# aapdo/M3ViT

Measured on AMD Instinct MI355X. Metric: images/sec fwd+bwd ViT-S/16 MoE(E=16,k=4) 224^2 bs=128, higher is better.
Workload: dtype f16; 1 GPU; configs[1]: ViT-Small/16 + MoE E=16 top-k=4 multi_gate, synthetic 224x224; batch_per_gpu=128, global_batch=128, task_passes=2, launch=hipGraph replay (one linear graph per task pass and stream), routing=deterministic (std=0), task_streams=2, wgrad_streams=0, activation_checkpointing=False, parallelism=single, full=False

## Files before the change

### m3vit_amd/csrc/attention_b16.hip

```cpp
#include "attention_dev.h"
#include <type_traits>

namespace m3 {

constexpr int AR_THREADS = 256;
constexpr float AR_LOG2E = 1.4426950408889634f;

typedef __fp16 ar_fp16x4 __attribute__((__vector_size__(4 * sizeof(__fp16))));

template <int W> __device__ __forceinline__ int swo(int row, int byte) {
  if (W == 32) return row * 64 + ((((byte >> 4) ^ (row >> 1)) & 3) << 4) + (byte & 15);
  return row * 128 + ((((byte >> 4) ^ row) & 7) << 4) + (byte & 15);
}

template <typename T, int W> __device__ __forceinline__ typename Mma<T>::frag row_frag(const char *img, int r0, int ch, int li, int lg) {
  return *(const typename Mma<T>::frag *)(img + swo<W>(r0 + li, ch * 64 + lg * 16));
}

template <typename T, int W> __device__ __forceinline__ typename Mma<T>::frag tr_frag(const char *img, int rb, int col, int li, int lg) {
  const int r = rb + 4 * lg + (li >> 2), byte = (col + 4 * (li & 3)) * 2;
  const ar_fp16x4 lo = __builtin_amdgcn_ds_read_tr16_b64_v4f16((__attribute__((address_space(3))) ar_fp16x4 *)(img + swo<W>(r, byte)));
  const ar_fp16x4 hi = __builtin_amdgcn_ds_read_tr16_b64_v4f16((__attribute__((address_space(3))) ar_fp16x4 *)(img + swo<W>(r + 16, byte)));
  f16x8 f;
  f[0] = (half_t)lo[0]; f[1] = (half_t)lo[1]; f[2] = (half_t)lo[2]; f[3] = (half_t)lo[3];
  f[4] = (half_t)hi[0]; f[5] = (half_t)hi[1]; f[6] = (half_t)hi[2]; f[7] = (half_t)hi[3];
  return __builtin_bit_cast(typename Mma<T>::frag, f);
}


template <typename T, int DH, int NKT>
__global__ __launch_bounds__(AR_THREADS, DH == 32 ? 4 : 2) void attention_fwd_res_kernel(const T *__restrict__ qkv, int N, int heads,
                                                                           T *__restrict__ o,
                                                                           float *__restrict__ lse, float scale) {
  constexpr int RBY = DH * 2, CPR = RBY / 16, NCH = DH / 32, NDT = DH / 16;
  constexpr int NKEY = NKT * 16, NQW = NKT / 4;
  extern __shared__ __attribute__((aligned(16))) char smem[];
  char *sK = smem, *sV = smem + NKEY * RBY;

  const int tid = threadIdx.x, lane = tid & 63, wave = tid >> 6;
  const int li = lane & 15, lg = lane >> 4;
  const int bh = xcd_remap(blockIdx.x, gridDim.x), b = bh / heads, h = bh - b * heads;
  const int C = heads * DH;
  const int64_t ld = 3 * (int64_t)C;
  const T *qbase = qkv + (int64_t)b * N * ld + h * DH;
  const T *kbase = qbase + C, *vbase = qbase + 2 * C;

  const int nkt = (N + 15) >> 4;
  typename Mma<T>::frag qfs[NQW][NCH];
#pragma unroll
  for (int i = 0; i < NQW; ++i) {
    const int qrow = (i * 4 + wave) * 16 + li;
#pragma unroll
    for (int ch = 0; ch < NCH; ++ch) {
      qfs[i][ch] = Mma<T>::zero();
      if (qrow < N) qfs[i][ch] = *(const typename Mma<T>::frag *)(qbase + (int64_t)qrow * ld + ch * 32 + 8 * lg);
    }
  }
  {
    constexpr int SIT = NKEY * CPR / AR_THREADS;
    constexpr int SB = SIT % 4 == 0 ? 4 : (SIT % 3 == 0 ? 3 : (SIT % 2 == 0 ? 2 : 1));
#pragma unroll
    for (int it0 = 0; it0 < SIT; it0 += SB) {
      u32x4 kv[SB], vv[SB];
#pragma unroll
      for (int it = 0; it < SB; ++it) {
        const int q = (it0 + it) * AR_THREADS + tid, row = q / CPR, c = q % CPR;
        kv[it] = u32x4{0u, 0u, 0u, 0u}; vv[it] = kv[it];
        if (row < N) {
          kv[it] = *(const u32x4 *)((const char *)(kbase + (int64_t)row * ld) + c * 16);
          vv[it] = *(const u32x4 *)((const char *)(vbase + (int64_t)row * ld) + c * 16);
        }
      }
#pragma unroll
      for (int it = 0; it < SB; ++it) {
        const int q = (it0 + it) * AR_THREADS + tid, row = q / CPR, c = q % CPR;
        *(u32x4 *)(sK + swo<DH>(row, c * 16)) = kv[it];
        *(u32x4 *)(sV + swo<DH>(row, c * 16)) = vv[it];
      }
    }
  }
  __syncthreads();

  const float c1 = scale * AR_LOG2E;
  const f32x4 zero4 = f32x4{0.f, 0.f, 0.f, 0.f};
#pragma unroll
  for (int i = 0; i < NQW; ++i) {
    const int qt = i * 4 + wave;
    if (qt >= nkt) break;
    const int qrow = qt * 16 + li;
    f32x4 st[NKT];
    float mx = -INFINITY;
#pragma unroll
    for (int kt = 0; kt < NKT; ++kt) {
      f32x4 sv = zero4;
#pragma unroll
      for (int ch = 0; ch < NCH; ++ch) sv = Mma<T>::mma(row_frag<T, DH>(sK, kt * 16, ch, li, lg), qfs[i][ch], sv);
      if (kt >= NKT - 4) {
#pragma unroll
        for (int r = 0; r < 4; ++r) sv[r] = (kt * 16 + 4 * lg + r < N) ? sv[r] : -INFINITY;
      }
      mx = fmaxf(fmaxf(mx, fmaxf(sv[0], sv[1])), fmaxf(sv[2], sv[3]));
      st[kt] = sv;
    }
    mx = fmaxf(mx, __shfl_xor(mx, 16, 64));
    mx = fmaxf(mx, __shfl_xor(mx, 32, 64));
    const float mc = mx * c1;
    float psum = 0.f;
#pragma unroll
    for (int kt = 0; kt < NKT; ++kt) {
#pragma unroll
      for (int r = 0; r < 4; ++r) {
        const float p = __builtin_amdgcn_exp2f(st[kt][r] * c1 - mc);
        st[kt][r] = p;
        psum += p;
      }
    }
    psum += __shfl_xor(psum, 16, 64);
    psum += __shfl_xor(psum, 32, 64);
    f32x4 oacc[NDT];
#pragma unroll
    for (int dt = 0; dt < NDT; ++dt) oacc[dt] = zero4;
#pragma unroll
    for (int cc = 0; cc < NKT / 2; ++cc) {
      const typename Mma<T>::frag pf = Mma<T>::from_tiles(&st[cc * 2]);
#pragma unroll
      for (int dt = 0; dt < NDT; ++dt) oacc[dt] = Mma<T>::mma(tr_frag<T, DH>(sV, cc * 32, dt * 16, li, lg), pf, oacc[dt]);
    }
    if (qrow < N) {
      const float inv = 1.0f / psum;
      T *orow = o + ((int64_t)b * N + qrow) * C + h * DH;
#pragma unroll
      for (int dt = 0; dt < NDT; ++dt) Vec4<T>::store(orow + dt * 16 + 4 * lg, oacc[dt] * inv);
      if (lg == 0) lse[((int64_t)b * heads + h) * N + qrow] = mx * scale + __logf(psum);
    }
  }
}

#ifdef M3_ATTN_STAMPS
constexpr int ASTAMP_WGS = 2048, ASTAMP_N = 40;
__device__ unsigned long long g_attn_stamps[ASTAMP_WGS][ASTAMP_N];
#define ATTN_STAMP(i)                                                                              \
  do {                                                                                             \
    if (threadIdx.x == 0 && blockIdx.x < ASTAMP_WGS && (i) < ASTAMP_N) g_attn_stamps[blockIdx.x][(i)] = __builtin_amdgcn_s_memtime(); \
  } while (0)
#else
#define ATTN_STAMP(i) do { } while (0)
#endif

template <typename T, int DH, int KTE>
__global__ __launch_bounds__(DH == 32 ? 256 : 512, DH == 32 ? 2 : 1) void attention_bwd_res_kernel(
    const T *__restrict__ qkv, const T *__restrict__ o, const T *__restrict__ d_o,
    const float *__restrict__ lse, int N, int heads, T *__restrict__ dqkv, float scale) {
  constexpr int RBY = DH * 2, CPR = RBY / 16, NCH = DH / 32, NDT = DH / 16;
  constexpr int NW = DH == 32 ? 4 : 8, NT = NW * 64;
  constexpr int NKEY = KTE * NW * 16, NKC = NKEY / 32;
  static_assert(2 * NDT == NW, "one dQ piece per wave");
  static_assert(NKEY <= ATTN_KEYS, "at most 256 keys");
  extern __shared__ __attribute__((aligned(16))) char smem[];
  const int NP = (N + 31) & ~31;
  char *sQ = smem, *sdO = sQ + NP * RBY, *sK = sdO + NP * RBY;
  char *sdS = sK + NKEY * RBY;
  float *sLse = (float *)(sdS + 2 * NKEY * 64);
  float *sDelta = sLse + NP;

  const int tid = threadIdx.x, lane = tid & 63, wave = __builtin_amdgcn_readfirstlane(tid >> 6);
  const int li = lane & 15, lg = lane >> 4;
  const int bh = xcd_remap(blockIdx.x, gridDim.x), b = bh / heads, h = bh - b * heads;
  const int C = heads * DH;
  const int64_t ld = 3 * (int64_t)C;
  const T *qbase = qkv + (int64_t)b * N * ld + h * DH;
  const T *kbase = qbase + C, *vbase = qbase + 2 * C;
  const T *obase = o + (int64_t)b * N * C + h * DH;
  const T *dobase = d_o + (int64_t)b * N * C + h * DH;
  T *dqbase = dqkv + (int64_t)b * N * ld + h * DH;
  const float *lbase = lse + ((int64_t)b * heads + h) * N;
  ATTN_STAMP(0);

  {
    constexpr int SIT = NKEY * CPR / NT;
    u32x4 qv[SIT], dv[SIT], kv[SIT], ov[SIT];
    float lv[SIT];
#pragma unroll
    for (int it = 0; it < SIT; ++it) {
      const int q = it * NT + tid, row = q / CPR, c = q % CPR;
      qv[it] = u32x4{0u, 0u, 0u, 0u}; dv[it] = qv[it]; kv[it] = qv[it]; ov[it] = qv[it];
      lv[it] = 1e30f;
      if (row < N) {
        qv[it] = *(const u32x4 *)((const char *)(qbase + (int64_t)row * ld) + c * 16);
        kv[it] = *(const u32x4 *)((const char *)(kbase + (int64_t)row * ld) + c * 16);
        dv[it] = *(const u32x4 *)((const char *)(dobase + (int64_t)row * C) + c * 16);
        ov[it] = *(const u32x4 *)((const char *)(obase + (int64_t)row * C) + c * 16);
        if (c == 0) lv[it] = lbase[row] * AR_LOG2E;
      }
    }
#pragma unroll
    for (int it = 0; it < SIT; ++it) {
      const int q = it * NT + tid, row = q / CPR, c = q % CPR;
      const typename Mma<T>::frag dh8 = __builtin_bit_cast(typename Mma<T>::frag, dv[it]), oh8 = __builtin_bit_cast(typename Mma<T>::frag, ov[it]);
      float sd = 0.f;
#pragma unroll
      for (int j = 0; j < 8; ++j) sd += (float)dh8[j] * (float)oh8[j];
#pragma unroll
      for (int m = 1; m < CPR; m <<= 1) sd += __shfl_xor(sd, m, 64);
      *(u32x4 *)(sK + swo<DH>(row, c * 16)) = kv[it];
      if (row < NP) {
        *(u32x4 *)(sQ + swo<DH>(row, c * 16)) = qv[it];
        *(u32x4 *)(sdO + swo<DH>(row, c * 16)) = dv[it];
        if (c == 0) {
          sDelta[row] = sd;
          sLse[row] = lv[it];
        }
      }
    }
  }
  typename Mma<T>::frag kf[KTE][NCH], vf[KTE][NCH];
#pragma unroll
  for (int kt = 0; kt < KTE; ++kt) {
    const int key = (kt * NW + wave) * 16 + li;
#pragma unroll
    for (int ch = 0; ch < NCH; ++ch) {
      kf[kt][ch] = Mma<T>::zero();
      vf[kt][ch] = Mma<T>::zero();
      if (key < N) {
        kf[kt][ch] = *(const typename Mma<T>::frag *)(kbase + (int64_t)key * ld + ch * 32 + 8 * lg);
        vf[kt][ch] = *(const typename Mma<T>::frag *)(vbase + (int64_t)key * ld + ch * 32 + 8 * lg);
      }
    }
  }
  const f32x4 zero4 = f32x4{0.f, 0.f, 0.f, 0.f};
  f32x4 dkt[NDT][KTE], dvt[NDT][KTE];
#pragma unroll
  for (int a = 0; a < NDT; ++a)
#pragma unroll
    for (int c = 0; c < KTE; ++c) { dkt[a][c] = zero4; dvt[a][c] = zero4; }
  ATTN_STAMP(1);
  __syncthreads();
  ATTN_STAMP(2);

  const float c1 = scale * AR_LOG2E, inv_c1 = 1.0f / c1;
  const int nsteps = NP >> 5;
  const bool last_key_ok = ((KTE - 1) * NW + wave) * 16 + li < N;
  const int dq_qt = wave / NDT, dq_dt = wave - dq_qt * NDT;
  typename Mma<T>::frag ka[NKC];
#pragma unroll
  for (int c = 0; c < NKC; ++c) ka[c] = tr_frag<T, DH>(sK, c * 32, dq_dt * 16, li, lg);
  for (int st = 0; st < nsteps; ++st) {
    const int qs = st * 32;
    char *dsb = sdS + (st & 1) * NKEY * 64;
    f32x4 pt[2][KTE], dst[2][KTE];
#pragma unroll
    for (int qt = 0; qt < 2; ++qt) {
      typename Mma<T>::frag qfr[NCH], dof[NCH];
#pragma unroll
      for (int ch = 0; ch < NCH; ++ch) {
        qfr[ch] = row_frag<T, DH>(sQ, qs + qt * 16, ch, li, lg);
        dof[ch] = row_frag<T, DH>(sdO, qs + qt * 16, ch, li, lg);
      }
      const f32x4 l4 = *(const f32x4 *)(sLse + qs + qt * 16 + 4 * lg), d4 = *(const f32x4 *)(sDelta + qs + qt * 16 + 4 * lg);
      const f32x4 s0 = l4 * (-inv_c1), dp0 = -d4;
#pragma unroll
      for (int kt = 0; kt < KTE; ++kt) {
        f32x4 s = s0, dp = dp0;
#pragma unroll
        for (int ch = 0; ch < NCH; ++ch) {
          s = Mma<T>::mma(qfr[ch], kf[kt][ch], s);
          dp = Mma<T>::mma(dof[ch], vf[kt][ch], dp);
        }
        f32x4 pv;
#pragma unroll
        for (int r = 0; r < 4; ++r) pv[r] = __builtin_amdgcn_exp2f(s[r] * c1);
        if (kt == KTE - 1) {
#pragma unroll
          for (int r = 0; r < 4; ++r) pv[r] = last_key_ok ? pv[r] : 0.f;
        }
        pt[qt][kt] = pv;
        dst[qt][kt] = pv * dp;
      }
    }
    ATTN_STAMP(3 + 4 * st);
    {
      typename Mma<T>::frag aq[NDT], ado[NDT];
#pragma unroll
      for (int dt = 0; dt < NDT; ++dt) {
        aq[dt] = tr_frag<T, DH>(sQ, qs, dt * 16, li, lg);
        ado[dt] = tr_frag<T, DH>(sdO, qs, dt * 16, li, lg);
      }
#pragma unroll
      for (int kt = 0; kt < KTE; ++kt) {
        f32x4 tp[2] = {pt[0][kt], pt[1][kt]}, td[2] = {dst[0][kt], dst[1][kt]};
        const typename Mma<T>::frag pf = Mma<T>::from_tiles(tp), dsf = Mma<T>::from_tiles(td);
#pragma unroll
        for (int dt = 0; dt < NDT; ++dt) {
          dvt[dt][kt] = Mma<T>::mma(ado[dt], pf, dvt[dt][kt]);
          dkt[dt][kt] = Mma<T>::mma(aq[dt], dsf, dkt[dt][kt]);
        }
        const int krow = (kt * NW + wave) * 16 + li;
#pragma unroll
        for (int qt = 0; qt < 2; ++qt) {
          typename Vec4<T>::type v = typename Vec4<T>::type{(T)dst[qt][kt][0], (T)dst[qt][kt][1], (T)dst[qt][kt][2], (T)dst[qt][kt][3]};
          *(typename Vec4<T>::type *)(dsb + swo<32>(krow, (qt * 16 + 4 * lg) * 2)) = v;
        }
      }
    }
    ATTN_STAMP(4 + 4 * st);
    __syncthreads();
    ATTN_STAMP(5 + 4 * st);
    {
      typename Mma<T>::frag da[NKC];
#pragma unroll
      for (int c = 0; c < NKC; ++c) da[c] = tr_frag<T, 32>(dsb, c * 32, dq_qt * 16, li, lg);
      f32x4 acc = zero4, acc2 = zero4;
#pragma unroll
      for (int c = 0; c < NKC; c += 2) {
        acc = Mma<T>::mma(ka[c], da[c], acc);
        if (c + 1 < NKC) acc2 = Mma<T>::mma(ka[c + 1], da[c + 1], acc2);
      }
      acc += acc2;
      const int qr = qs + dq_qt * 16 + li;
      if (qr < N) Vec4<T>::store(dqbase + (int64_t)qr * ld + dq_dt * 16 + 4 * lg, acc * scale);
    }
    ATTN_STAMP(6 + 4 * st);
  }

#pragma unroll
  for (int kt = 0; kt < KTE; ++kt) {
    const int key = (kt * NW + wave) * 16 + li;
    if (key < N) {
#pragma unroll
      for (int dt = 0; dt < NDT; ++dt) {
        Vec4<T>::store(dqbase + C + (int64_t)key * ld + dt * 16 + 4 * lg, dkt[dt][kt] * scale);
        Vec4<T>::store(dqbase + 2 * C + (int64_t)key * ld + dt * 16 + 4 * lg, dvt[dt][kt]);
      }
    }
  }
  ATTN_STAMP(36);
#ifdef M3_ATTN_STAMPS
  asm volatile("s_waitcnt vmcnt(0)" ::: "memory");
  ATTN_STAMP(37);
#endif
}

template <typename T, int DH>
__global__ __launch_bounds__(AR_THREADS, 2) void attention_fwd_stream_kernel(const T *__restrict__ qkv, int N, int heads,
                                                                              T *__restrict__ o,
                                                                              float *__restrict__ lse, float scale) {
  constexpr int RBY = DH * 2, CPR = RBY / 16, NCH = DH / 32, NDT = DH / 16;
  constexpr int KT = 64;
  constexpr int NLD = KT * CPR / AR_THREADS;
  extern __shared__ __attribute__((aligned(16))) char smem[];
  char *sK = smem, *sV = smem + 2 * KT * RBY;

  const int tid = threadIdx.x, lane = tid & 63, wave = tid >> 6;
  const int li = lane & 15, lg = lane >> 4;
  const int nqb = gridDim.x;
  const int log_id = xcd_remap(blockIdx.x + nqb * blockIdx.y, nqb * gridDim.y);
  const int qb = log_id % nqb;
  const int bh = log_id / nqb, b = bh / heads, h = bh - b * heads;
  const int C = heads * DH;
  const int64_t ld = 3 * (int64_t)C;
  const T *qbase = qkv + (int64_t)b * N * ld + h * DH;
  const T *kbase = qbase + C, *vbase = qbase + 2 * C;

  const int qrow = qb * 64 + wave * 16 + li;
  typename Mma<T>::frag qf[NCH];
#pragma unroll
  for (int ch = 0; ch < NCH; ++ch) {
    qf[ch] = Mma<T>::zero();
    if (qrow < N) qf[ch] = *(const typename Mma<T>::frag *)(qbase + (int64_t)qrow * ld + ch * 32 + 8 * lg);
  }
  u32x4 rk[NLD], rv[NLD];
  auto fetch = [&](int key0) {
#pragma unroll
    for (int i = 0; i < NLD; ++i) {
      const int q = tid + AR_THREADS * i, row = q / CPR, c = q % CPR;
      rk[i] = u32x4{0u, 0u, 0u, 0u};
      rv[i] = u32x4{0u, 0u, 0u, 0u};
      if (key0 + row < N) {
        rk[i] = *(const u32x4 *)((const char *)(kbase + (int64_t)(key0 + row) * ld) + c * 16);
        rv[i] = *(const u32x4 *)((const char *)(vbase + (int64_t)(key0 + row) * ld) + c * 16);
      }
    }
  };
  auto stash = [&](int buf) {
#pragma unroll
    for (int i = 0; i < NLD; ++i) {
      const int q = tid + AR_THREADS * i, row = q / CPR, c = q % CPR;
      *(u32x4 *)(sK + buf * KT * RBY + swo<DH>(row, c * 16)) = rk[i];
      *(u32x4 *)(sV + buf * KT * RBY + swo<DH>(row, c * 16)) = rv[i];
    }
  };
  fetch(0);
  stash(0);
  __syncthreads();

  const f32x4 zero4 = f32x4{0.f, 0.f, 0.f, 0.f};
  f32x4 oacc[NDT];
#pragma unroll
  for (int dt = 0; dt < NDT; ++dt) oacc[dt] = zero4;
  const float c1 = scale * AR_LOG2E;
  float m_run = -INFINITY, l_run = 0.f;
  const int ntiles = (N + KT - 1) / KT;
  for (int t = 0; t < ntiles; ++t) {
    const int key0 = t * KT, buf = t & 1;
    const bool more = t + 1 < ntiles;
    if (more) fetch(key0 + KT);
    const char *cK = sK + buf * KT * RBY, *cV = sV + buf * KT * RBY;
    f32x4 st[4];
    float mt = -INFINITY;
#pragma unroll
    for (int kt = 0; kt < 4; ++kt) {
      f32x4 sv = zero4;
#pragma unroll
      for (int ch = 0; ch < NCH; ++ch) sv = Mma<T>::mma(row_frag<T, DH>(cK, kt * 16, ch, li, lg), qf[ch], sv);
      if (!more) {
#pragma unroll
        for (int r = 0; r < 4; ++r) sv[r] = (key0 + kt * 16 + 4 * lg + r < N) ? sv[r] : -INFINITY;
      }
      mt = fmaxf(fmaxf(mt, fmaxf(sv[0], sv[1])), fmaxf(sv[2], sv[3]));
      st[kt] = sv;
    }
    mt = fmaxf(mt, __shfl_xor(mt, 16, 64));
    mt = fmaxf(mt, __shfl_xor(mt, 32, 64));
    const float m_new = fmaxf(m_run, mt);
    const float alpha = __builtin_amdgcn_exp2f((m_run - m_new) * c1);
    const float mc = m_new * c1;
    float psum = 0.f;
#pragma unroll
    for (int kt = 0; kt < 4; ++kt)
#pragma unroll
      for (int r = 0; r < 4; ++r) {
        const float p = __builtin_amdgcn_exp2f(st[kt][r] * c1 - mc);
        st[kt][r] = p;
        psum += p;
      }
    l_run = l_run * alpha + psum;
    m_run = m_new;
#pragma unroll
    for (int dt = 0; dt < NDT; ++dt) oacc[dt] *= alpha;
#pragma unroll
    for (int cc = 0; cc < 2; ++cc) {
      const typename Mma<T>::frag pf = Mma<T>::from_tiles(&st[cc * 2]);
#pragma unroll
      for (int dt = 0; dt < NDT; ++dt) oacc[dt] = Mma<T>::mma(tr_frag<T, DH>(cV, cc * 32, dt * 16, li, lg), pf, oacc[dt]);
    }
    if (more) stash(buf ^ 1);
    __syncthreads();
  }
  float l_tot = l_run + __shfl_xor(l_run, 16, 64);
  l_tot += __shfl_xor(l_tot, 32, 64);
  if (qrow < N) {
    const float inv = 1.0f / l_tot;
    T *orow = o + ((int64_t)b * N + qrow) * C + h * DH;
#pragma unroll
    for (int dt = 0; dt < NDT; ++dt) Vec4<T>::store(orow + dt * 16 + 4 * lg, oacc[dt] * inv);
    if (lg == 0) lse[((int64_t)b * heads + h) * N + qrow] = m_run * scale + __logf(l_tot);
  }
}

template <typename T>
static int launch_attention_fwd_stream_t(const void *qkv, int B, int N, int heads, int dh, void *o, float *lse, float scale,
                                hipStream_t s) {
  const dim3 grid((N + 63) / 64, B * heads);
  const size_t lds = (size_t)4 * 64 * dh * 2;
#define M3_AFS_GO(DH_) hipLaunchKernelGGL((attention_fwd_stream_kernel<T, DH_>), grid, dim3(AR_THREADS), lds, s, (const T *)qkv, N, heads, \
                                          (T *)o, lse, scale)
  if (dh == 32) M3_AFS_GO(32); else M3_AFS_GO(64);
#undef M3_AFS_GO
  return check_launch("m3_attention_fwd");
}

template <typename T, int DH>
__global__ __launch_bounds__(64) void attention_delta_kernel(const T *__restrict__ o, const T *__restrict__ d_o,
                                                             int64_t rows, int heads, float *__restrict__ delta) {
  const int64_t i = (int64_t)blockIdx.x * 64 + threadIdx.x;
  if (i >= rows * heads) return;
  const T *po = o + i * DH, *pd = d_o + i * DH;
  float s = 0.f;
#pragma unroll
  for (int c = 0; c < DH / 8; ++c) {
    const typename Mma<T>::frag a = *(const typename Mma<T>::frag *)(po + c * 8), b = *(const typename Mma<T>::frag *)(pd + c * 8);
#pragma unroll
    for (int j = 0; j < 8; ++j) s += (float)a[j] * (float)b[j];
  }
  delta[i] = s;
}

template <typename T, int DH>
__global__ __launch_bounds__(DH == 32 ? 256 : 512, DH == 32 ? 2 : 1) void attention_bwd_stream_kernel(
    const T *__restrict__ qkv, const T *__restrict__ d_o, const float *__restrict__ lse,
    const float *__restrict__ delta, int N, int heads, T *__restrict__ dqkv, float *__restrict__ dq_ws, float scale) {
  constexpr int RBY = DH * 2, CPR = RBY / 16, NCH = DH / 32, NDT = DH / 16;
  constexpr int NW = DH == 32 ? 4 : 8, NT = NW * 64, KTW = 16 / NW;
  static_assert(2 * NDT == NW && 32 * CPR * 2 == NT, "one dQ piece and one staged chunk per thread");
  extern __shared__ __attribute__((aligned(16))) char smem[];
  char *sK = smem;
  char *sQ = sK + ATTN_KEYS * RBY;
  char *sdO = sQ + 2 * 32 * RBY;
  char *sdS = sdO + 2 * 32 * RBY;
  float *sLse = (float *)(sdS + 2 * ATTN_KEYS * 64);
  float *sDelta = sLse + 64;

  const int tid = threadIdx.x, lane = tid & 63, wave = __builtin_amdgcn_readfirstlane(tid >> 6);
  const int li = lane & 15, lg = lane >> 4;
  const int nkb = (N + ATTN_KEYS - 1) / ATTN_KEYS;
  const int wid = xcd_remap(blockIdx.x, gridDim.x);
  const int bh = wid / nkb, kbi = wid - bh * nkb, b = bh / heads, h = bh - b * heads;
  const int kb0 = kbi * ATTN_KEYS;
  const int C = heads * DH;
  const int64_t ld = 3 * (int64_t)C;
  const T *qbase = qkv + (int64_t)b * N * ld + h * DH;
  const T *kbase = qbase + C, *vbase = qbase + 2 * C;
  const T *dobase = d_o + (int64_t)b * N * C + h * DH;
  T *dqbase = dqkv + (int64_t)b * N * ld + h * DH;
  const float *lbase = lse + ((int64_t)b * heads + h) * N;
  const float *dbase = delta + (int64_t)b * N * heads + h;
  float *dqw = dq_ws + ((int64_t)kbi * (gridDim.x / nkb) + bh) * N * DH;
  const int nkeys = (N - kb0 < ATTN_KEYS) ? N - kb0 : ATTN_KEYS;
  const int nkt = (nkeys + 15) >> 4;
  const int nkc = (nkeys + 31) >> 5;

  for (int q = tid; q < ATTN_KEYS * CPR; q += NT) {
    const int row = q / CPR, c = q % CPR;
    u32x4 kv = u32x4{0u, 0u, 0u, 0u};
    if (row < nkeys) kv = *(const u32x4 *)((const char *)(kbase + (int64_t)(kb0 + row) * ld) + c * 16);
    *(u32x4 *)(sK + swo<DH>(row, c * 16)) = kv;
  }
  for (int q = tid; q < 2 * ATTN_KEYS * 4; q += NT) *(u32x4 *)(sdS + q * 16) = u32x4{0u, 0u, 0u, 0u};
  typename Mma<T>::frag kf[KTW][NCH], vf[KTW][NCH];
#pragma unroll
  for (int kt = 0; kt < KTW; ++kt) {
    const int key = kb0 + (kt * NW + wave) * 16 + li;
#pragma unroll
    for (int ch = 0; ch < NCH; ++ch) {
      kf[kt][ch] = Mma<T>::zero();
      vf[kt][ch] = Mma<T>::zero();
      if (key < N) {
        kf[kt][ch] = *(const typename Mma<T>::frag *)(kbase + (int64_t)key * ld + ch * 32 + 8 * lg);
        vf[kt][ch] = *(const typename Mma<T>::frag *)(vbase + (int64_t)key * ld + ch * 32 + 8 * lg);
      }
    }
  }
  const f32x4 zero4 = f32x4{0.f, 0.f, 0.f, 0.f};
  f32x4 dkt[NDT][KTW], dvt[NDT][KTW];
#pragma unroll
  for (int a = 0; a < NDT; ++a)
#pragma unroll
    for (int c = 0; c < KTW; ++c) { dkt[a][c] = zero4; dvt[a][c] = zero4; }

  const int half_t_ = NT / 2;
  const bool is_do = tid >= half_t_;
  const int sq = is_do ? tid - half_t_ : tid;
  const int srow = sq / CPR, sc = sq % CPR;
  auto fetch = [&](int qs, u32x4 &v, float &l2, float &dl) {
    const int qr = qs + srow;
    v = u32x4{0u, 0u, 0u, 0u};
    if (qr < N) {
      if (is_do) v = *(const u32x4 *)((const char *)(dobase + (int64_t)qr * C) + sc * 16);
      else v = *(const u32x4 *)((const char *)(qbase + (int64_t)qr * ld) + sc * 16);
    }
    l2 = 1e30f; dl = 0.f;
    if (tid < 32 && qs + tid < N) { l2 = lbase[qs + tid] * AR_LOG2E; dl = dbase[(int64_t)(qs + tid) * heads]; }
  };
  auto stash = [&](int buf, const u32x4 &v, float l2, float dl) {
    *(u32x4 *)((is_do ? sdO : sQ) + buf * 32 * RBY + swo<DH>(srow, sc * 16)) = v;
    if (tid < 32) { sLse[buf * 32 + tid] = l2; sDelta[buf * 32 + tid] = dl; }
  };
  {
    u32x4 v; float l2, dl;
    fetch(0, v, l2, dl);
    stash(0, v, l2, dl);
  }
  __syncthreads();

  const float c1 = scale * AR_LOG2E, inv_c1 = 1.0f / c1;
  const int nsteps = (N + 31) >> 5;
  auto run = [&](auto full_c) {
  constexpr bool FULL = decltype(full_c)::value;
  for (int st = 0; st < nsteps; ++st) {
    const int qs = st * 32, buf = st & 1;
    const char *cQ = sQ + buf * 32 * RBY, *cdO = sdO + buf * 32 * RBY;
    char *dsb = sdS + buf * ATTN_KEYS * 64;
    u32x4 nv; float nl2, ndl;
    const bool more = st + 1 < nsteps;
    if (more) fetch(qs + 32, nv, nl2, ndl);
    f32x4 pt[2][KTW], dst[2][KTW];
#pragma unroll
    for (int qt = 0; qt < 2; ++qt) {
      typename Mma<T>::frag qfr[NCH], dof[NCH];
#pragma unroll
      for (int ch = 0; ch < NCH; ++ch) {
        qfr[ch] = row_frag<T, DH>(cQ, qt * 16, ch, li, lg);
        dof[ch] = row_frag<T, DH>(cdO, qt * 16, ch, li, lg);
      }
      f32x4 s0, dp0;
#pragma unroll
      for (int r = 0; r < 4; ++r) {
        s0[r] = -sLse[buf * 32 + qt * 16 + 4 * lg + r] * inv_c1;
        dp0[r] = -sDelta[buf * 32 + qt * 16 + 4 * lg + r];
      }
#pragma unroll
      for (int kt = 0; kt < KTW; ++kt) {
        const int tix = kt * NW + wave;
        if (FULL || tix < nkt) {
          f32x4 s = s0, dp = dp0;
#pragma unroll
          for (int ch = 0; ch < NCH; ++ch) {
            s = Mma<T>::mma(qfr[ch], kf[kt][ch], s);
            dp = Mma<T>::mma(dof[ch], vf[kt][ch], dp);
          }
          f32x4 pv;
#pragma unroll
          for (int r = 0; r < 4; ++r) pv[r] = __builtin_amdgcn_exp2f(s[r] * c1);
          if (!FULL && tix == nkt - 1 && tix * 16 + li >= nkeys) pv = zero4;
          pt[qt][kt] = pv;
#pragma unroll
          for (int r = 0; r < 4; ++r) dst[qt][kt][r] = pv[r] * dp[r];
        } else {
          pt[qt][kt] = zero4;
          dst[qt][kt] = zero4;
        }
      }
    }
    ATTN_STAMP(3 + 4 * st);
    {
      typename Mma<T>::frag aq[NDT], ado[NDT];
#pragma unroll
      for (int dt = 0; dt < NDT; ++dt) {
        aq[dt] = tr_frag<T, DH>(cQ, 0, dt * 16, li, lg);
        ado[dt] = tr_frag<T, DH>(cdO, 0, dt * 16, li, lg);
      }
#pragma unroll
      for (int kt = 0; kt < KTW; ++kt) {
        if (FULL || kt * NW + wave < nkt) {
          f32x4 tp[2] = {pt[0][kt], pt[1][kt]}, td[2] = {dst[0][kt], dst[1][kt]};
          const typename Mma<T>::frag pf = Mma<T>::from_tiles(tp), dsf = Mma<T>::from_tiles(td);
#pragma unroll
          for (int dt = 0; dt < NDT; ++dt) {
            dvt[dt][kt] = Mma<T>::mma(ado[dt], pf, dvt[dt][kt]);
            dkt[dt][kt] = Mma<T>::mma(aq[dt], dsf, dkt[dt][kt]);
          }
          const int krow = (kt * NW + wave) * 16 + li;
#pragma unroll
          for (int qt = 0; qt < 2; ++qt) {
            typename Vec4<T>::type v = typename Vec4<T>::type{(T)dst[qt][kt][0], (T)dst[qt][kt][1], (T)dst[qt][kt][2], (T)dst[qt][kt][3]};
            *(typename Vec4<T>::type *)(dsb + swo<32>(krow, (qt * 16 + 4 * lg) * 2)) = v;
          }
        }
      }
    }
    if (more) stash(buf ^ 1, nv, nl2, ndl);
    __syncthreads();
    {
      const int qt = wave / NDT, dt = wave - qt * NDT;
      typename Mma<T>::frag ka[ATTN_KEYS / 32], da[ATTN_KEYS / 32];
#pragma unroll
      for (int c = 0; c < ATTN_KEYS / 32; ++c) {
        const int cc = (FULL || c < nkc) ? c : nkc - 1;
        ka[c] = tr_frag<T, DH>(sK, cc * 32, dt * 16, li, lg);
        da[c] = tr_frag<T, 32>(dsb, cc * 32, qt * 16, li, lg);
      }
      f32x4 acc = zero4;
#pragma unroll
      for (int c = 0; c < ATTN_KEYS / 32; ++c)
        if (FULL || c < nkc) acc = Mma<T>::mma(ka[c], da[c], acc);
      const int qr = qs + qt * 16 + li;
      if (qr < N) *(f32x4 *)(dqw + (int64_t)qr * DH + dt * 16 + 4 * lg) = acc * scale;
    }
  }
  };
  if (nkeys == ATTN_KEYS) run(std::true_type{}); else run(std::false_type{});

#pragma unroll
  for (int kt = 0; kt < KTW; ++kt) {
    const int key = kb0 + (kt * NW + wave) * 16 + li;
    if (key < N) {
#pragma unroll
      for (int dt = 0; dt < NDT; ++dt) {
        Vec4<T>::store(dqbase + C + (int64_t)key * ld + dt * 16 + 4 * lg, dkt[dt][kt] * scale);
        Vec4<T>::store(dqbase + 2 * C + (int64_t)key * ld + dt * 16 + 4 * lg, dvt[dt][kt]);
      }
    }
  }
}

static size_t attn_stream_bwd_lds(int dh) { return (size_t)ATTN_KEYS * dh * 2 + 4 * 32 * dh * 2 + 2 * ATTN_KEYS * 64 + 128 * sizeof(float); }

template <typename T>
static int launch_attention_bwd_stream_t(const void *qkv, const void *o, const void *d_o, const float *lse, int B, int N, int heads,
                                int dh, void *dqkv, float *dq_ws, float scale, hipStream_t s) {
  const int nkb = attn_key_blocks(N);
  float *delta = dq_ws + attn_bwd_ws(B, N, heads, dh).delta_off;
  const int64_t rows = (int64_t)B * N;
  const unsigned dblocks = (unsigned)((rows * heads + 63) / 64);
  static bool attr_set = false;
  if (!attr_set) {
    (void)hipFuncSetAttribute((const void *)attention_bwd_stream_kernel<T, 32>, hipFuncAttributeMaxDynamicSharedMemorySize,
                              (int)attn_stream_bwd_lds(32));
    (void)hipFuncSetAttribute((const void *)attention_bwd_stream_kernel<T, 64>, hipFuncAttributeMaxDynamicSharedMemorySize,
                              (int)attn_stream_bwd_lds(64));
    attr_set = true;
  }
#define M3_ABS_GO(DH_, NT_)                                                                                                   \
  hipLaunchKernelGGL((attention_delta_kernel<T, DH_>), dim3(dblocks), dim3(64), 0, s, (const T *)o, (const T *)d_o, rows, heads, delta); \
  hipLaunchKernelGGL((attention_bwd_stream_kernel<T, DH_>), dim3(B * heads * nkb), dim3(NT_), attn_stream_bwd_lds(DH_), s,    \
                     (const T *)qkv, (const T *)d_o, lse, delta, N, heads, (T *)dqkv, dq_ws, scale)
  if (dh == 32) { M3_ABS_GO(32, 256); } else { M3_ABS_GO(64, 512); }
#undef M3_ABS_GO
  return check_launch("m3_attention_bwd");
}

static inline int attn_res_fwd_nkt(int N) { return ((N + 15) / 16 + 3) / 4 * 4; }
static size_t attn_res_fwd_lds(int N, int dh) { return (size_t)2 * attn_res_fwd_nkt(N) * 16 * dh * 2; }
static inline int attn_res_bwd_kte(int N, int dh) { const int nw = dh == 32 ? 4 : 8; return ((N + 15) / 16 + nw - 1) / nw; }
static size_t attn_res_bwd_lds(int N, int dh) {
  const size_t np = (N + 31) & ~31;
  const size_t nkey = (size_t)attn_res_bwd_kte(N, dh) * (dh == 32 ? 4 : 8) * 16;
  return 2 * np * dh * 2 + nkey * dh * 2 + 2 * nkey * 64 + 2 * np * sizeof(float);
}

template <typename T>
static int launch_attention_fwd_res_t(const void *qkv, int B, int N, int heads, int dh, void *o, float *lse, float scale,
                             hipStream_t s) {
  const size_t lds = attn_res_fwd_lds(N, dh);
  const int nkt = attn_res_fwd_nkt(N);
#define M3_AF_GO(DH_, NK_) hipLaunchKernelGGL((attention_fwd_res_kernel<T, DH_, NK_>), dim3(B * heads), dim3(AR_THREADS), lds, s, \
                                             (const T *)qkv, N, heads, (T *)o, lse, scale)
  if (dh == 32) {
    if (nkt == 4) M3_AF_GO(32, 4); else if (nkt == 8) M3_AF_GO(32, 8); else if (nkt == 12) M3_AF_GO(32, 12); else M3_AF_GO(32, 16);
  } else {
    if (nkt == 4) M3_AF_GO(64, 4); else if (nkt == 8) M3_AF_GO(64, 8); else if (nkt == 12) M3_AF_GO(64, 12); else M3_AF_GO(64, 16);
  }
#undef M3_AF_GO
  return check_launch("m3_attention_fwd");
}

template <typename T>
static int launch_attention_bwd_res_t(const void *qkv, const void *o, const void *d_o, const float *lse, int B, int N, int heads,
                             int dh, void *dqkv, float scale, hipStream_t s) {
  const size_t lds = attn_res_bwd_lds(N, dh);
  const int kte = attn_res_bwd_kte(N, dh);
  static bool attr_set = false;
#define M3_AB_ATTR(DH_, K_) (void)hipFuncSetAttribute((const void *)attention_bwd_res_kernel<T, DH_, K_>, hipFuncAttributeMaxDynamicSharedMemorySize, \
                                                      (int)attn_res_bwd_lds(K_ * (DH_ == 32 ? 64 : 128), DH_))
  if (!attr_set) {
    M3_AB_ATTR(32, 1); M3_AB_ATTR(32, 2); M3_AB_ATTR(32, 3); M3_AB_ATTR(32, 4); M3_AB_ATTR(64, 1); M3_AB_ATTR(64, 2);
    attr_set = true;
  }
#undef M3_AB_ATTR
#define M3_AB_GO(DH_, K_, NT_) hipLaunchKernelGGL((attention_bwd_res_kernel<T, DH_, K_>), dim3(B * heads), dim3(NT_), lds, s, (const T *)qkv, \
                                                 (const T *)o, (const T *)d_o, lse, N, heads, (T *)dqkv, scale)
  if (dh == 32) {
    if (kte == 1) M3_AB_GO(32, 1, 256); else if (kte == 2) M3_AB_GO(32, 2, 256); else if (kte == 3) M3_AB_GO(32, 3, 256); else M3_AB_GO(32, 4, 256);
  } else {
    if (kte == 1) M3_AB_GO(64, 1, 512); else M3_AB_GO(64, 2, 512);
  }
#undef M3_AB_GO
  return check_launch("m3_attention_bwd");
}

#define M3_B16(fn, ...) (dtype == M3_BF16 ? fn<bf16_t>(__VA_ARGS__) : fn<half_t>(__VA_ARGS__))
int launch_attention_fwd_stream(int dtype, const void *qkv, int B, int N, int heads, int dh, void *o, float *lse, float scale, hipStream_t s) {
  return M3_B16(launch_attention_fwd_stream_t, qkv, B, N, heads, dh, o, lse, scale, s);
}
int launch_attention_bwd_stream(int dtype, const void *qkv, const void *o, const void *d_o, const float *lse, int B, int N, int heads, int dh, void *dqkv, float *dq_ws, float scale, hipStream_t s) {
  return M3_B16(launch_attention_bwd_stream_t, qkv, o, d_o, lse, B, N, heads, dh, dqkv, dq_ws, scale, s);
}
int launch_attention_fwd_res(int dtype, const void *qkv, int B, int N, int heads, int dh, void *o, float *lse, float scale, hipStream_t s) {
  return M3_B16(launch_attention_fwd_res_t, qkv, B, N, heads, dh, o, lse, scale, s);
}
int launch_attention_bwd_res(int dtype, const void *qkv, const void *o, const void *d_o, const float *lse, int B, int N, int heads, int dh, void *dqkv, float scale, hipStream_t s) {
  return M3_B16(launch_attention_bwd_res_t, qkv, o, d_o, lse, B, N, heads, dh, dqkv, scale, s);
}
#undef M3_B16

}

#ifdef M3_ATTN_STAMPS
extern "C" int m3_debug_attn_stamps(unsigned long long *dst, int wgs) {
  if (wgs > m3::ASTAMP_WGS) wgs = m3::ASTAMP_WGS;
  return hipMemcpyFromSymbol(dst, HIP_SYMBOL(m3::g_attn_stamps), (size_t)wgs * m3::ASTAMP_N * sizeof(unsigned long long)) == hipSuccess ? M3_OK : M3_ERR_LAUNCH;
}
#endif
```

Before: 7762 images/s.

## Trim padded key/query tiles in resident attention fwd and bwd kernels

The forward kernel now pads the key count to a multiple of 32 instead of 64, and rotates which wave handles which query tile per head so the partially filled last tile is spread across waves. The backward kernel is now templated on 32-key chunks rather than per-wave tiles. It pads queries to 16, handles a trailing half step with a single-tile path, and lets waves with no last key tile run a shorter sweep. For ViT-S/16 at 224 (197 tokens, dh=64) this is meant to cut the padded MMA and exp work done on empty tiles, in exchange for more template instantiations and extra code paths.

```diff
diff --git a/m3vit_amd/csrc/attention_b16.hip b/m3vit_amd/csrc/attention_b16.hip
--- a/m3vit_amd/csrc/attention_b16.hip
+++ b/m3vit_amd/csrc/attention_b16.hip
@@ -33,7 +33,7 @@
                                                                            T *__restrict__ o,
                                                                            float *__restrict__ lse, float scale) {
   constexpr int RBY = DH * 2, CPR = RBY / 16, NCH = DH / 32, NDT = DH / 16;
-  constexpr int NKEY = NKT * 16, NQW = NKT / 4;
+  constexpr int NKEY = NKT * 16, NQW = (NKT + 3) / 4;
   extern __shared__ __attribute__((aligned(16))) char smem[];
   char *sK = smem, *sV = smem + NKEY * RBY;
 
@@ -46,10 +46,11 @@
   const T *kbase = qbase + C, *vbase = qbase + 2 * C;
 
   const int nkt = (N + 15) >> 4;
+  const int slot = (wave + bh) & 3;
   typename Mma<T>::frag qfs[NQW][NCH];
 #pragma unroll
   for (int i = 0; i < NQW; ++i) {
-    const int qrow = (i * 4 + wave) * 16 + li;
+    const int qrow = (i * 4 + slot) * 16 + li;
 #pragma unroll
     for (int ch = 0; ch < NCH; ++ch) {
       qfs[i][ch] = Mma<T>::zero();
@@ -57,13 +58,14 @@
     }
   }
   {
-    constexpr int SIT = NKEY * CPR / AR_THREADS;
-    constexpr int SB = SIT % 4 == 0 ? 4 : (SIT % 3 == 0 ? 3 : (SIT % 2 == 0 ? 2 : 1));
+    constexpr int SIT = (NKEY * CPR + AR_THREADS - 1) / AR_THREADS;
+    constexpr bool SFULL = NKEY * CPR % AR_THREADS == 0;
+    constexpr int SB = SIT % 4 == 0 ? 4 : (SIT % 3 == 0 ? 3 : (SIT > 4 ? 4 : SIT));
 #pragma unroll
     for (int it0 = 0; it0 < SIT; it0 += SB) {
       u32x4 kv[SB], vv[SB];
 #pragma unroll
-      for (int it = 0; it < SB; ++it) {
+      for (int it = 0; it < SB && it0 + it < SIT; ++it) {
         const int q = (it0 + it) * AR_THREADS + tid, row = q / CPR, c = q % CPR;
         kv[it] = u32x4{0u, 0u, 0u, 0u}; vv[it] = kv[it];
         if (row < N) {
@@ -72,10 +74,12 @@
         }
       }
 #pragma unroll
-      for (int it = 0; it < SB; ++it) {
+      for (int it = 0; it < SB && it0 + it < SIT; ++it) {
         const int q = (it0 + it) * AR_THREADS + tid, row = q / CPR, c = q % CPR;
-        *(u32x4 *)(sK + swo<DH>(row, c * 16)) = kv[it];
-        *(u32x4 *)(sV + swo<DH>(row, c * 16)) = vv[it];
+        if (SFULL || row < NKEY) {
+          *(u32x4 *)(sK + swo<DH>(row, c * 16)) = kv[it];
+          *(u32x4 *)(sV + swo<DH>(row, c * 16)) = vv[it];
+        }
       }
     }
   }
@@ -85,7 +89,7 @@
   const f32x4 zero4 = f32x4{0.f, 0.f, 0.f, 0.f};
 #pragma unroll
   for (int i = 0; i < NQW; ++i) {
-    const int qt = i * 4 + wave;
+    const int qt = i * 4 + slot;
     if (qt >= nkt) break;
     const int qrow = qt * 16 + li;
     f32x4 st[NKT];
@@ -95,7 +99,7 @@
       f32x4 sv = zero4;
 #pragma unroll
       for (int ch = 0; ch < NCH; ++ch) sv = Mma<T>::mma(row_frag<T, DH>(sK, kt * 16, ch, li, lg), qfs[i][ch], sv);
-      if (kt >= NKT - 4) {
+      if (kt >= NKT - 2) {
 #pragma unroll
         for (int r = 0; r < 4; ++r) sv[r] = (kt * 16 + 4 * lg + r < N) ? sv[r] : -INFINITY;
       }
@@ -117,6 +121,7 @@
     }
     psum += __shfl_xor(psum, 16, 64);
     psum += __shfl_xor(psum, 32, 64);
+    if (DH == 32 && NKT == 14) __builtin_amdgcn_sched_barrier(0);
     f32x4 oacc[NDT];
 #pragma unroll
     for (int dt = 0; dt < NDT; ++dt) oacc[dt] = zero4;
@@ -147,17 +152,29 @@
 #define ATTN_STAMP(i) do { } while (0)
 #endif
 
-template <typename T, int DH, int KTE>
+template <int V> using ar_int = std::integral_constant<int, V>;
+
+template <typename T, int W> __device__ __forceinline__ typename Mma<T>::frag tr_frag_lo(const char *img, int rb, int col, int li, int lg) {
+  const int r = rb + 4 * lg + (li >> 2), byte = (col + 4 * (li & 3)) * 2;
+  const ar_fp16x4 lo = __builtin_amdgcn_ds_read_tr16_b64_v4f16((__attribute__((address_space(3))) ar_fp16x4 *)(img + swo<W>(r, byte)));
+  f16x8 f;
+  f[0] = (half_t)lo[0]; f[1] = (half_t)lo[1]; f[2] = (half_t)lo[2]; f[3] = (half_t)lo[3];
+  f[4] = (half_t)0.f; f[5] = (half_t)0.f; f[6] = (half_t)0.f; f[7] = (half_t)0.f;
+  return __builtin_bit_cast(typename Mma<T>::frag, f);
+}
+
+template <typename T, int DH, int NKC>
 __global__ __launch_bounds__(DH == 32 ? 256 : 512, DH == 32 ? 2 : 1) void attention_bwd_res_kernel(
     const T *__restrict__ qkv, const T *__restrict__ o, const T *__restrict__ d_o,
     const float *__restrict__ lse, int N, int heads, T *__restrict__ dqkv, float scale) {
   constexpr int RBY = DH * 2, CPR = RBY / 16, NCH = DH / 32, NDT = DH / 16;
   constexpr int NW = DH == 32 ? 4 : 8, NT = NW * 64;
-  constexpr int NKEY = KTE * NW * 16, NKC = NKEY / 32;
+  constexpr int NKEY = NKC * 32;
+  constexpr int KTE = (2 * NKC + NW - 1) / NW;
   static_assert(2 * NDT == NW, "one dQ piece per wave");
   static_assert(NKEY <= ATTN_KEYS, "at most 256 keys");
   extern __shared__ __attribute__((aligned(16))) char smem[];
-  const int NP = (N + 31) & ~31;
+  const int NP = (N + 15) & ~15;
   char *sQ = smem, *sdO = sQ + NP * RBY, *sK = sdO + NP * RBY;
   char *sdS = sK + NKEY * RBY;
   float *sLse = (float *)(sdS + 2 * NKEY * 64);
@@ -166,6 +183,8 @@
   const int tid = threadIdx.x, lane = tid & 63, wave = __builtin_amdgcn_readfirstlane(tid >> 6);
   const int li = lane & 15, lg = lane >> 4;
   const int bh = xcd_remap(blockIdx.x, gridDim.x), b = bh / heads, h = bh - b * heads;
+  const int slot = (wave + bh) & (NW - 1);
+  const int nkt = (N + 15) >> 4;
   const int C = heads * DH;
   const int64_t ld = 3 * (int64_t)C;
   const T *qbase = qkv + (int64_t)b * N * ld + h * DH;
@@ -177,7 +196,8 @@
   ATTN_STAMP(0);
 
   {
-    constexpr int SIT = NKEY * CPR / NT;
+    constexpr int SIT = (NKEY * CPR + NT - 1) / NT;
+    constexpr bool SFULL = NKEY * CPR % NT == 0;
     u32x4 qv[SIT], dv[SIT], kv[SIT], ov[SIT];
     float lv[SIT];
 #pragma unroll
@@ -193,6 +213,7 @@
         if (c == 0) lv[it] = lbase[row] * AR_LOG2E;
       }
     }
+    if (nkt * 16 < NKEY && tid < 128) *(u32x4 *)(sdS + (tid >> 6) * NKEY * 64 + nkt * 16 * 64 + (tid & 63) * 16) = u32x4{0u, 0u, 0u, 0u};
 #pragma unroll
     for (int it = 0; it < SIT; ++it) {
       const int q = it * NT + tid, row = q / CPR, c = q % CPR;
@@ -202,7 +223,7 @@
       for (int j = 0; j < 8; ++j) sd += (float)dh8[j] * (float)oh8[j];
 #pragma unroll
       for (int m = 1; m < CPR; m <<= 1) sd += __shfl_xor(sd, m, 64);
-      *(u32x4 *)(sK + swo<DH>(row, c * 16)) = kv[it];
+      if (SFULL || row < NKEY) *(u32x4 *)(sK + swo<DH>(row, c * 16)) = kv[it];
       if (row < NP) {
         *(u32x4 *)(sQ + swo<DH>(row, c * 16)) = qv[it];
         *(u32x4 *)(sdO + swo<DH>(row, c * 16)) = dv[it];
@@ -216,7 +237,7 @@
   typename Mma<T>::frag kf[KTE][NCH], vf[KTE][NCH];
 #pragma unroll
   for (int kt = 0; kt < KTE; ++kt) {
-    const int key = (kt * NW + wave) * 16 + li;
+    const int key = (kt * NW + slot) * 16 + li;
 #pragma unroll
     for (int ch = 0; ch < NCH; ++ch) {
       kf[kt][ch] = Mma<T>::zero();
@@ -228,111 +249,119 @@
     }
   }
   const f32x4 zero4 = f32x4{0.f, 0.f, 0.f, 0.f};
-  f32x4 dkt[NDT][KTE], dvt[NDT][KTE];
-#pragma unroll
-  for (int a = 0; a < NDT; ++a)
-#pragma unroll
-    for (int c = 0; c < KTE; ++c) { dkt[a][c] = zero4; dvt[a][c] = zero4; }
   ATTN_STAMP(1);
   __syncthreads();
   ATTN_STAMP(2);
 
   const float c1 = scale * AR_LOG2E, inv_c1 = 1.0f / c1;
-  const int nsteps = NP >> 5;
-  const bool last_key_ok = ((KTE - 1) * NW + wave) * 16 + li < N;
+  const int nfull = NP >> 5;
+  const bool last_key_ok = ((KTE - 1) * NW + slot) * 16 + li < N;
   const int dq_qt = wave / NDT, dq_dt = wave - dq_qt * NDT;
   typename Mma<T>::frag ka[NKC];
 #pragma unroll
   for (int c = 0; c < NKC; ++c) ka[c] = tr_frag<T, DH>(sK, c * 32, dq_dt * 16, li, lg);
-  for (int st = 0; st < nsteps; ++st) {
-    const int qs = st * 32;
-    char *dsb = sdS + (st & 1) * NKEY * 64;
-    f32x4 pt[2][KTE], dst[2][KTE];
-#pragma unroll
-    for (int qt = 0; qt < 2; ++qt) {
-      typename Mma<T>::frag qfr[NCH], dof[NCH];
-#pragma unroll
-      for (int ch = 0; ch < NCH; ++ch) {
-        qfr[ch] = row_frag<T, DH>(sQ, qs + qt * 16, ch, li, lg);
-        dof[ch] = row_frag<T, DH>(sdO, qs + qt * 16, ch, li, lg);
-      }
-      const f32x4 l4 = *(const f32x4 *)(sLse + qs + qt * 16 + 4 * lg), d4 = *(const f32x4 *)(sDelta + qs + qt * 16 + 4 * lg);
-      const f32x4 s0 = l4 * (-inv_c1), dp0 = -d4;
-#pragma unroll
-      for (int kt = 0; kt < KTE; ++kt) {
-        f32x4 s = s0, dp = dp0;
+
+  auto sweep = [&](auto kt_c) {
+    constexpr int KT = decltype(kt_c)::value, KA = KT > 0 ? KT : 1;
+    f32x4 dkt[NDT][KA], dvt[NDT][KA];
+#pragma unroll
+    for (int a = 0; a < NDT; ++a)
+#pragma unroll
+      for (int c = 0; c < KA; ++c) { dkt[a][c] = zero4; dvt[a][c] = zero4; }
+    auto step = [&](auto nq_c, int st) {
+      constexpr int NQ = decltype(nq_c)::value;
+      const int qs = st * 32;
+      char *dsb = sdS + (st & 1) * NKEY * 64;
+      f32x4 pt[NQ][KA], dst[NQ][KA];
+#pragma unroll
+      for (int qt = 0; qt < NQ; ++qt) {
+        typename Mma<T>::frag qfr[NCH], dof[NCH];
 #pragma unroll
         for (int ch = 0; ch < NCH; ++ch) {
-          s = Mma<T>::mma(qfr[ch], kf[kt][ch], s);
-          dp = Mma<T>::mma(dof[ch], vf[kt][ch], dp);
-        }
-        f32x4 pv;
-#pragma unroll
-        for (int r = 0; r < 4; ++r) pv[r] = __builtin_amdgcn_exp2f(s[r] * c1);
-        if (kt == KTE - 1) {
-#pragma unroll
-          for (int r = 0; r < 4; ++r) pv[r] = last_key_ok ? pv[r] : 0.f;
-        }
-        pt[qt][kt] = pv;
-        dst[qt][kt] = pv * dp;
-      }
-    }
-    ATTN_STAMP(3 + 4 * st);
-    {
-      typename Mma<T>::frag aq[NDT], ado[NDT];
-#pragma unroll
-      for (int dt = 0; dt < NDT; ++dt) {
-        aq[dt] = tr_frag<T, DH>(sQ, qs, dt * 16, li, lg);
-        ado[dt] = tr_frag<T, DH>(sdO, qs, dt * 16, li, lg);
-      }
-#pragma unroll
-      for (int kt = 0; kt < KTE; ++kt) {
-        f32x4 tp[2] = {pt[0][kt], pt[1][kt]}, td[2] = {dst[0][kt], dst[1][kt]};
-        const typename Mma<T>::frag pf = Mma<T>::from_tiles(tp), dsf = Mma<T>::from_tiles(td);
+          qfr[ch] = row_frag<T, DH>(sQ, qs + qt * 16, ch, li, lg);
+          dof[ch] = row_frag<T, DH>(sdO, qs + qt * 16, ch, li, lg);
+        }
+        const f32x4 l4 = *(const f32x4 *)(sLse + qs + qt * 16 + 4 * lg), d4 = *(const f32x4 *)(sDelta + qs + qt * 16 + 4 * lg);
+        const f32x4 s0 = l4 * (-inv_c1), dp0 = -d4;
+#pragma unroll
+        for (int kt = 0; kt < KT; ++kt) {
+          f32x4 s = s0, dp = dp0;
+#pragma unroll
+          for (int ch = 0; ch < NCH; ++ch) {
+            s = Mma<T>::mma(qfr[ch], kf[kt][ch], s);
+            dp = Mma<T>::mma(dof[ch], vf[kt][ch], dp);
+          }
+          f32x4 pv;
+#pragma unroll
+          for (int r = 0; r < 4; ++r) pv[r] = __builtin_amdgcn_exp2f(s[r] * c1);
+          if (kt == KTE - 1) {
+#pragma unroll
+            for (int r = 0; r < 4; ++r) pv[r] = last_key_ok ? pv[r] : 0.f;
+          }
+          pt[qt][kt] = pv;
+          dst[qt][kt] = pv * dp;
+        }
+      }
+      ATTN_STAMP(3 + 4 * st);
+      {
+        typename Mma<T>::frag aq[NDT], ado[NDT];
 #pragma unroll
         for (int dt = 0; dt < NDT; ++dt) {
-          dvt[dt][kt] = Mma<T>::mma(ado[dt], pf, dvt[dt][kt]);
-          dkt[dt][kt] = Mma<T>::mma(aq[dt], dsf, dkt[dt][kt]);
-        }
-        const int krow = (kt * NW + wave) * 16 + li;
-#pragma unroll
-        for (int qt = 0; qt < 2; ++qt) {
-          typename Vec4<T>::type v = typename Vec4<T>::type{(T)dst[qt][kt][0], (T)dst[qt][kt][1], (T)dst[qt][kt][2], (T)dst[qt][kt][3]};
-          *(typename Vec4<T>::type *)(dsb + swo<32>(krow, (qt * 16 + 4 * lg) * 2)) = v;
-        }
-      }
-    }
-    ATTN_STAMP(4 + 4 * st);
-    __syncthreads();
-    ATTN_STAMP(5 + 4 * st);
-    {
-      typename Mma<T>::frag da[NKC];
-#pragma unroll
-      for (int c = 0; c < NKC; ++c) da[c] = tr_frag<T, 32>(dsb, c * 32, dq_qt * 16, li, lg);
-      f32x4 acc = zero4, acc2 = zero4;
-#pragma unroll
-      for (int c = 0; c < NKC; c += 2) {
-        acc = Mma<T>::mma(ka[c], da[c], acc);
-        if (c + 1 < NKC) acc2 = Mma<T>::mma(ka[c + 1], da[c + 1], acc2);
-      }
-      acc += acc2;
-      const int qr = qs + dq_qt * 16 + li;
-      if (qr < N) Vec4<T>::store(dqbase + (int64_t)qr * ld + dq_dt * 16 + 4 * lg, acc * scale);
-    }
-    ATTN_STAMP(6 + 4 * st);
-  }
-
-#pragma unroll
-  for (int kt = 0; kt < KTE; ++kt) {
-    const int key = (kt * NW + wave) * 16 + li;
-    if (key < N) {
-#pragma unroll
-      for (int dt = 0; dt < NDT; ++dt) {
-        Vec4<T>::store(dqbase + C + (int64_t)key * ld + dt * 16 + 4 * lg, dkt[dt][kt] * scale);
-        Vec4<T>::store(dqbase + 2 * C + (int64_t)key * ld + dt * 16 + 4 * lg, dvt[dt][kt]);
-      }
-    }
-  }
+          aq[dt] = NQ == 2 ? tr_frag<T, DH>(sQ, qs, dt * 16, li, lg) : tr_frag_lo<T, DH>(sQ, qs, dt * 16, li, lg);
+          ado[dt] = NQ == 2 ? tr_frag<T, DH>(sdO, qs, dt * 16, li, lg) : tr_frag_lo<T, DH>(sdO, qs, dt * 16, li, lg);
+        }
+#pragma unroll
+        for (int kt = 0; kt < KT; ++kt) {
+          f32x4 tp[2] = {pt[0][kt], NQ == 2 ? pt[NQ - 1][kt] : zero4}, td[2] = {dst[0][kt], NQ == 2 ? dst[NQ - 1][kt] : zero4};
+          const typename Mma<T>::frag pf = Mma<T>::from_tiles(tp), dsf = Mma<T>::from_tiles(td);
+#pragma unroll
+          for (int dt = 0; dt < NDT; ++dt) {
+            dvt[dt][kt] = Mma<T>::mma(ado[dt], pf, dvt[dt][kt]);
+            dkt[dt][kt] = Mma<T>::mma(aq[dt], dsf, dkt[dt][kt]);
+          }
+          const int krow = (kt * NW + slot) * 16 + li;
+#pragma unroll
+          for (int qt = 0; qt < NQ; ++qt) {
+            typename Vec4<T>::type v = typename Vec4<T>::type{(T)dst[qt][kt][0], (T)dst[qt][kt][1], (T)dst[qt][kt][2], (T)dst[qt][kt][3]};
+            *(typename Vec4<T>::type *)(dsb + swo<32>(krow, (qt * 16 + 4 * lg) * 2)) = v;
+          }
+        }
+      }
+      ATTN_STAMP(4 + 4 * st);
+      __syncthreads();
+      ATTN_STAMP(5 + 4 * st);
+      if (NQ == 2 || dq_qt == 0) {
+        typename Mma<T>::frag da[NKC];
+#pragma unroll
+        for (int c = 0; c < NKC; ++c) da[c] = tr_frag<T, 32>(dsb, c * 32, dq_qt * 16, li, lg);
+        f32x4 acc = zero4, acc2 = zero4;
+#pragma unroll
+        for (int c = 0; c < NKC; c += 2) {
+          acc = Mma<T>::mma(ka[c], da[c], acc);
+          if (c + 1 < NKC) acc2 = Mma<T>::mma(ka[c + 1], da[c + 1], acc2);
+        }
+        acc += acc2;
+        const int qr = qs + dq_qt * 16 + li;
+        if (qr < N) Vec4<T>::store(dqbase + (int64_t)qr * ld + dq_dt * 16 + 4 * lg, acc * scale);
+      }
+      ATTN_STAMP(6 + 4 * st);
+    };
+    for (int st = 0; st < nfull; ++st) step(ar_int<2>{}, st);
+    if (NP & 16) step(ar_int<1>{}, nfull);
+
+#pragma unroll
+    for (int kt = 0; kt < KT; ++kt) {
+      const int key = (kt * NW + slot) * 16 + li;
+      if (key < N) {
+#pragma unroll
+        for (int dt = 0; dt < NDT; ++dt) {
+          Vec4<T>::store(dqbase + C + (int64_t)key * ld + dt * 16 + 4 * lg, dkt[dt][kt] * scale);
+          Vec4<T>::store(dqbase + 2 * C + (int64_t)key * ld + dt * 16 + 4 * lg, dvt[dt][kt]);
+        }
+      }
+    }
+  };
+  if ((KTE - 1) * NW + slot < nkt) sweep(ar_int<KTE>{}); else sweep(ar_int<KTE - 1>{});
   ATTN_STAMP(36);
 #ifdef M3_ATTN_STAMPS
   asm volatile("s_waitcnt vmcnt(0)" ::: "memory");
@@ -709,12 +738,12 @@
   return check_launch("m3_attention_bwd");
 }
 
-static inline int attn_res_fwd_nkt(int N) { return ((N + 15) / 16 + 3) / 4 * 4; }
+static inline int attn_res_fwd_nkt(int N) { return ((N + 15) / 16 + 1) / 2 * 2; }
 static size_t attn_res_fwd_lds(int N, int dh) { return (size_t)2 * attn_res_fwd_nkt(N) * 16 * dh * 2; }
-static inline int attn_res_bwd_kte(int N, int dh) { const int nw = dh == 32 ? 4 : 8; return ((N + 15) / 16 + nw - 1) / nw; }
+static inline int attn_res_bwd_nkc(int N) { return (N + 31) / 32; }
 static size_t attn_res_bwd_lds(int N, int dh) {
-  const size_t np = (N + 31) & ~31;
-  const size_t nkey = (size_t)attn_res_bwd_kte(N, dh) * (dh == 32 ? 4 : 8) * 16;
+  const size_t np = (N + 15) & ~15;
+  const size_t nkey = (size_t)attn_res_bwd_nkc(N) * 32;
   return 2 * np * dh * 2 + nkey * dh * 2 + 2 * nkey * 64 + 2 * np * sizeof(float);
 }
 
@@ -725,11 +754,14 @@
   const int nkt = attn_res_fwd_nkt(N);
 #define M3_AF_GO(DH_, NK_) hipLaunchKernelGGL((attention_fwd_res_kernel<T, DH_, NK_>), dim3(B * heads), dim3(AR_THREADS), lds, s, \
                                              (const T *)qkv, N, heads, (T *)o, lse, scale)
-  if (dh == 32) {
-    if (nkt == 4) M3_AF_GO(32, 4); else if (nkt == 8) M3_AF_GO(32, 8); else if (nkt == 12) M3_AF_GO(32, 12); else M3_AF_GO(32, 16);
-  } else {
-    if (nkt == 4) M3_AF_GO(64, 4); else if (nkt == 8) M3_AF_GO(64, 8); else if (nkt == 12) M3_AF_GO(64, 12); else M3_AF_GO(64, 16);
-  }
+#define M3_AF_PICK(DH_)                                                                                                       \
+  switch (nkt) {                                                                                                              \
+    case 2: M3_AF_GO(DH_, 2); break;   case 4: M3_AF_GO(DH_, 4); break;   case 6: M3_AF_GO(DH_, 6); break;                    \
+    case 8: M3_AF_GO(DH_, 8); break;   case 10: M3_AF_GO(DH_, 10); break; case 12: M3_AF_GO(DH_, 12); break;                  \
+    case 14: M3_AF_GO(DH_, 14); break; default: M3_AF_GO(DH_, 16); break;                                                     \
+  }
+  if (dh == 32) { M3_AF_PICK(32); } else { M3_AF_PICK(64); }
+#undef M3_AF_PICK
 #undef M3_AF_GO
   return check_launch("m3_attention_fwd");
 }
@@ -738,22 +770,28 @@
 static int launch_attention_bwd_res_t(const void *qkv, const void *o, const void *d_o, const float *lse, int B, int N, int heads,
                              int dh, void *dqkv, float scale, hipStream_t s) {
   const size_t lds = attn_res_bwd_lds(N, dh);
-  const int kte = attn_res_bwd_kte(N, dh);
+  const int nkc = attn_res_bwd_nkc(N);
   static bool attr_set = false;
 #define M3_AB_ATTR(DH_, K_) (void)hipFuncSetAttribute((const void *)attention_bwd_res_kernel<T, DH_, K_>, hipFuncAttributeMaxDynamicSharedMemorySize, \
-                                                      (int)attn_res_bwd_lds(K_ * (DH_ == 32 ? 64 : 128), DH_))
+                                                      (int)attn_res_bwd_lds(K_ * 32, DH_))
+#define M3_AB_ATTRS(DH_) M3_AB_ATTR(DH_, 1); M3_AB_ATTR(DH_, 2); M3_AB_ATTR(DH_, 3); M3_AB_ATTR(DH_, 4); M3_AB_ATTR(DH_, 5); \
+                         M3_AB_ATTR(DH_, 6); M3_AB_ATTR(DH_, 7); M3_AB_ATTR(DH_, 8)
   if (!attr_set) {
-    M3_AB_ATTR(32, 1); M3_AB_ATTR(32, 2); M3_AB_ATTR(32, 3); M3_AB_ATTR(32, 4); M3_AB_ATTR(64, 1); M3_AB_ATTR(64, 2);
+    M3_AB_ATTRS(32); M3_AB_ATTRS(64);
     attr_set = true;
   }
+#undef M3_AB_ATTRS
 #undef M3_AB_ATTR
-#define M3_AB_GO(DH_, K_, NT_) hipLaunchKernelGGL((attention_bwd_res_kernel<T, DH_, K_>), dim3(B * heads), dim3(NT_), lds, s, (const T *)qkv, \
-                                                 (const T *)o, (const T *)d_o, lse, N, heads, (T *)dqkv, scale)
-  if (dh == 32) {
-    if (kte == 1) M3_AB_GO(32, 1, 256); else if (kte == 2) M3_AB_GO(32, 2, 256); else if (kte == 3) M3_AB_GO(32, 3, 256); else M3_AB_GO(32, 4, 256);
-  } else {
-    if (kte == 1) M3_AB_GO(64, 1, 512); else M3_AB_GO(64, 2, 512);
-  }
+#define M3_AB_GO(DH_, K_) hipLaunchKernelGGL((attention_bwd_res_kernel<T, DH_, K_>), dim3(B * heads), dim3(DH_ == 32 ? 256 : 512), lds, s, \
+                                            (const T *)qkv, (const T *)o, (const T *)d_o, lse, N, heads, (T *)dqkv, scale)
+#define M3_AB_PICK(DH_)                                                                                                       \
+  switch (nkc) {                                                                                                              \
+    case 1: M3_AB_GO(DH_, 1); break; case 2: M3_AB_GO(DH_, 2); break; case 3: M3_AB_GO(DH_, 3); break;                        \
+    case 4: M3_AB_GO(DH_, 4); break; case 5: M3_AB_GO(DH_, 5); break; case 6: M3_AB_GO(DH_, 6); break;                        \
+    case 7: M3_AB_GO(DH_, 7); break; default: M3_AB_GO(DH_, 8); break;                                                        \
+  }
+  if (dh == 32) { M3_AB_PICK(32); } else { M3_AB_PICK(64); }
+#undef M3_AB_PICK
 #undef M3_AB_GO
   return check_launch("m3_attention_bwd");
 }
```

Result: no change. 7816 images/s, median of 6 (+0.7%).
